# mbzuai-metaverse/XMem2

Hardware: AMD Instinct MI355X
Metric: frames/sec at 480p, 1 obj, 32 memory frames; mask IoU vs reference (higher is better)
Workload: dtype f32

## Files before the change

### include/xmem_hip.h

```cpp
#ifndef XMEM_HIP_H
#define XMEM_HIP_H

#include <stddef.h>
#include <stdint.h>

#ifdef __cplusplus
extern "C" {
#endif

typedef enum {
    XMEM_OK = 0,
    XMEM_ERR_BAD_ARG = -1,
    XMEM_ERR_UNSUPPORTED = -2,
    XMEM_ERR_WORKSPACE = -3,
    XMEM_ERR_LAUNCH = -4,
    XMEM_ERR_TOPK = -5
} xmem_status;

#define XMEM_ABI_VERSION 4
int xmem_version(void);
const char* xmem_last_error_string(int code);

int xmem_trace_marker(int tag, void* stream);

// ... 29 lines not shown
    int stream, ring;
} xmem_conv_plan_info;
int xmem_conv2d_plan_info(const xmem_conv_desc* d, xmem_conv_plan_info* out);

int xmem_conv2d_nhwc(const xmem_conv_desc* d, void* workspace, size_t workspace_bytes, void* stream);

#define XMEM_DILATED_NO_TAP_SKIP 1
size_t xmem_conv2d_dilated_workspace_bytes(const xmem_conv_desc* d, int dilation);
int xmem_conv2d_nhwc_dilated(const xmem_conv_desc* d, int dilation, int flags, void* workspace, size_t workspace_bytes, void* stream);

enum { XMEM_AUG_BRIGHTNESS = 0, XMEM_AUG_POSTERIZE = 1, XMEM_AUG_GRAY = 2, XMEM_AUG_SHARPNESS = 3, XMEM_AUG_BLUR7 = 4, XMEM_AUG_AFFINE = 5 };
#define XMEM_AUG_MAX 32
typedef struct {
    int type;
    float factor;
    double image_matrix[6];
    float mask_grid[6];
} xmem_aug_desc;
size_t xmem_augment_workspace_bytes(int n_aug, int H, int W);
int xmem_augment_frames(const uint8_t* img, const float* mask, int H, int W, int K, const xmem_aug_desc* descs, int n_aug,
                        uint8_t* out_img, float* out_mask, void* workspace, size_t workspace_bytes, void* stream);

int xmem_maxpool3x3s2(const float* in, float* out, int B, int H, int W, int C, void* stream);

int xmem_upsample2x_add(const float* g, const float* skip, float* out, int B, int h, int w, int C, void* stream);

int xmem_area_downsample(const float* in, int ldin, float* out, int ldout, int B, int H, int W, int C, int r, void* stream);

int xmem_copy_channels(const float* src, int ldsrc, int srcB, float* dst, int lddst, int B, int P, int C, void* stream);

int xmem_hidden_update_gather(const float* g16, int c16, const float* g8, int c8, const float* g4, int c4, const float* logits,
                              float* out, int ldout, int K, int h, int w, void* stream);

size_t xmem_cbam_workspace_bytes(int B, int P, int C);
int xmem_cbam_residual(const float* g, float* out, int B, int H, int W, int C,
                       const float* w1, const float* b1, const float* w2, const float* b2,
                       const float* sw, const float* sb, void* workspace, size_t workspace_bytes, void* stream);

int xmem_gru_gate(const float* values, const float* h, float* new_h, int B, int P, int Ch, void* stream);

int xmem_add3(const float* a, const float* b, const float* c, float* y, size_t n, void* stream);

int xmem_maxpool3x3s2_t(const void* in, int in_half, void* out, int out_half, int B, int H, int W, int C, void* stream);
int xmem_upsample2x_add_t(const void* g, const void* skip, void* out, int half, int B, int h, int w, int C, void* stream);
int xmem_area_downsample_t(const void* in, int in_half, int ldin, void* out, int out_half, int ldout, int B, int H, int W, int C, int r, void* stream);
int xmem_copy_channels_t(const void* src, int src_half, int ldsrc, int srcB, void* dst, int dst_half, int lddst, int B, int P, int C, void* stream);
int xmem_cbam_residual_t(const void* g, void* out, int half, int B, int H, int W, int C,
                         const float* w1, const float* b1, const float* w2, const float* b2,
                         const float* sw, const float* sb, void* workspace, size_t workspace_bytes, void* stream);
int xmem_gru_gate_t(const void* values, int values_half, const float* h, float* new_h, int B, int P, int Ch, void* stream);

int xmem_pack_image(const float* img, float* out, int H, int W, int Hp, int Wp, int lh, int lw, void* stream);

int xmem_pack_image_u8(const uint8_t* img, float* out, int H, int W, int Hp, int Wp, int lh, int lw,
                       const float* mean3_host, const float* std3_host, void* stream);

int xmem_pack_value_input(const float* image4, const float* masks, float* out, int K, int Hp, int Wp, void* stream);

int xmem_key_post(const float* proj, int ldp, float* key, float* shrinkage, float* selection, int P, int Ck, void* stream);

int xmem_logits_to_prob(const float* logits, float* prob, float* prob_padded, int K, int h4, int w4,
                        int H, int W, int lh, int lw, void* stream);

int xmem_aggregate_masks(const float* masks, float* prob, int K, int H, int W, void* stream);

int xmem_merge_masks(const float* pred_no_bg, const float* mask, uint64_t valid_bits, float* out, int K, int H, int W, void* stream);
// ... 106 lines not shown
```

### xmem2_amd/_lib.py

```python
import ctypes as C
import os

import torch

_HERE = os.path.dirname(os.path.abspath(__file__))
LIB_PATH = os.path.join(_HERE, 'csrc', 'libxmem_hip.so')
_lib = None

c_float_p = C.c_void_p
c_void_p = C.c_void_p


ABI_VERSION = 4


class ConvDesc(C.Structure):
    _fields_ = [('inp', C.c_void_p), ('B', C.c_int), ('H', C.c_int), ('W', C.c_int), ('Cin', C.c_int), ('ldin', C.c_int),
                ('w', C.c_void_p), ('Cout', C.c_int), ('KH', C.c_int), ('KW', C.c_int), ('stride', C.c_int), ('pad', C.c_int),
                ('scale', C.c_void_p), ('shift', C.c_void_p),
                ('res', C.c_void_p), ('ldres', C.c_int),
                ('out', C.c_void_p), ('ldout', C.c_int),
                ('relu_in', C.c_int), ('relu_out', C.c_int), ('plan_tile', C.c_int), ('plan_splitk', C.c_int), ('w_winograd', C.c_void_p),
                ('res_broadcast', C.c_int), ('w_winograd_f16', C.c_void_p), ('w_winograd4', C.c_void_p),
                ('arith', C.c_int), ('w_split', C.c_void_p), ('w_winograd_split', C.c_void_p), ('w_winograd4_split', C.c_void_p),
# ... 18 lines not shown


class AffinityHint(C.Structure):
    _fields_ = [('idx', C.c_void_p), ('top_k', C.c_int), ('n_seg', C.c_int), ('seg_n', C.c_int * 4), ('grid_w', C.c_int)]


class ValueSegment(C.Structure):
    _fields_ = [('value', C.c_void_p), ('n', C.c_int)]


_SIGS = {
    'xmem_version': (C.c_int, []),
    'xmem_last_error_string': (C.c_char_p, [C.c_int]),
    'xmem_trace_marker': (C.c_int, [C.c_int, C.c_void_p]),
    'xmem_conv2d_workspace_bytes': (C.c_size_t, [C.POINTER(ConvDesc)]),
    'xmem_conv2d_plan_info': (C.c_int, [C.POINTER(ConvDesc), C.POINTER(ConvPlanInfo)]),
    'xmem_conv2d_nhwc': (C.c_int, [C.POINTER(ConvDesc), C.c_void_p, C.c_size_t, C.c_void_p]),
    'xmem_conv2d_dilated_workspace_bytes': (C.c_size_t, [C.POINTER(ConvDesc), C.c_int]),
    'xmem_conv2d_nhwc_dilated': (C.c_int, [C.POINTER(ConvDesc), C.c_int, C.c_int, C.c_void_p, C.c_size_t, C.c_void_p]),
    'xmem_maxpool3x3s2': (C.c_int, [C.c_void_p, C.c_void_p, C.c_int, C.c_int, C.c_int, C.c_int, C.c_void_p]),
    'xmem_maxpool3x3s2_t': (C.c_int, [C.c_void_p, C.c_int, C.c_void_p, C.c_int, C.c_int, C.c_int, C.c_int, C.c_int, C.c_void_p]),
    'xmem_upsample2x_add_t': (C.c_int, [C.c_void_p, C.c_void_p, C.c_void_p, C.c_int, C.c_int, C.c_int, C.c_int, C.c_int, C.c_void_p]),
    'xmem_area_downsample_t': (C.c_int, [C.c_void_p, C.c_int, C.c_int, C.c_void_p, C.c_int, C.c_int, C.c_int, C.c_int, C.c_int, C.c_int, C.c_int, C.c_void_p]),
    'xmem_copy_channels_t': (C.c_int, [C.c_void_p, C.c_int, C.c_int, C.c_int, C.c_void_p, C.c_int, C.c_int, C.c_int, C.c_int, C.c_int, C.c_void_p]),
    'xmem_cbam_residual_t': (C.c_int, [C.c_void_p, C.c_void_p, C.c_int, C.c_int, C.c_int, C.c_int, C.c_int,
                                       C.c_void_p, C.c_void_p, C.c_void_p, C.c_void_p, C.c_void_p, C.c_void_p,
                                       C.c_void_p, C.c_size_t, C.c_void_p]),
    'xmem_gru_gate_t': (C.c_int, [C.c_void_p, C.c_int, C.c_void_p, C.c_void_p, C.c_int, C.c_int, C.c_int, C.c_void_p]),
    'xmem_upsample2x_add': (C.c_int, [C.c_void_p, C.c_void_p, C.c_void_p, C.c_int, C.c_int, C.c_int, C.c_int, C.c_void_p]),
    'xmem_area_downsample': (C.c_int, [C.c_void_p, C.c_int, C.c_void_p, C.c_int, C.c_int, C.c_int, C.c_int, C.c_int, C.c_int, C.c_void_p]),
    'xmem_copy_channels': (C.c_int, [C.c_void_p, C.c_int, C.c_int, C.c_void_p, C.c_int, C.c_int, C.c_int, C.c_int, C.c_void_p]),
    'xmem_hidden_update_gather': (C.c_int, [C.c_void_p, C.c_int, C.c_void_p, C.c_int, C.c_void_p, C.c_int, C.c_void_p, C.c_void_p, C.c_int, C.c_int, C.c_int,
                                            C.c_int, C.c_void_p]),
    'xmem_cbam_workspace_bytes': (C.c_size_t, [C.c_int, C.c_int, C.c_int]),
    'xmem_cbam_residual': (C.c_int, [C.c_void_p, C.c_void_p, C.c_int, C.c_int, C.c_int, C.c_int,
                                     C.c_void_p, C.c_void_p, C.c_void_p, C.c_void_p, C.c_void_p, C.c_void_p,
                                     C.c_void_p, C.c_size_t, C.c_void_p]),
    'xmem_gru_gate': (C.c_int, [C.c_void_p, C.c_void_p, C.c_void_p, C.c_int, C.c_int, C.c_int, C.c_void_p]),
    'xmem_add3': (C.c_int, [C.c_void_p, C.c_void_p, C.c_void_p, C.c_void_p, C.c_size_t, C.c_void_p]),
    'xmem_pack_image': (C.c_int, [C.c_void_p, C.c_void_p, C.c_int, C.c_int, C.c_int, C.c_int, C.c_int, C.c_int, C.c_void_p]),
    'xmem_pack_image_u8': (C.c_int, [C.c_void_p, C.c_void_p, C.c_int, C.c_int, C.c_int, C.c_int, C.c_int, C.c_int,
                                     C.POINTER(C.c_float), C.POINTER(C.c_float), C.c_void_p]),
    'xmem_pack_value_input': (C.c_int, [C.c_void_p, C.c_void_p, C.c_void_p, C.c_int, C.c_int, C.c_int, C.c_void_p]),
    'xmem_key_post': (C.c_int, [C.c_void_p, C.c_int, C.c_void_p, C.c_void_p, C.c_void_p, C.c_int, C.c_int, C.c_void_p]),
    'xmem_logits_to_prob': (C.c_int, [C.c_void_p, C.c_void_p, C.c_void_p, C.c_int, C.c_int, C.c_int, C.c_int, C.c_int, C.c_int, C.c_int, C.c_void_p]),
    'xmem_aggregate_masks': (C.c_int, [C.c_void_p, C.c_void_p, C.c_int, C.c_int, C.c_int, C.c_void_p]),
    'xmem_merge_masks': (C.c_int, [C.c_void_p, C.c_void_p, C.c_uint64, C.c_void_p, C.c_int, C.c_int, C.c_int, C.c_void_p]),
    'xmem_resize_bilinear': (C.c_int, [C.c_void_p, C.c_void_p, C.c_int, C.c_int, C.c_int, C.c_int, C.c_int, C.c_void_p]),
    'xmem_argmax_u8': (C.c_int, [C.c_void_p, C.c_void_p, C.c_int, C.c_int, C.c_int, C.c_void_p]),
    'xmem_ensemble_accumulate': (C.c_int, [C.c_void_p, C.c_int, C.c_int, C.c_int, C.c_int, C.c_void_p, C.c_int, C.c_int, C.c_int,
                                           C.c_void_p, C.c_void_p]),
    'xmem_jf_counts': (C.c_int, [C.c_void_p, C.c_void_p, C.c_void_p, C.c_int, C.c_int, C.c_int, C.c_int, C.c_void_p, C.c_void_p]),
    'xmem_s2m_pack': (C.c_int, [C.c_void_p, C.c_void_p, C.c_void_p, C.c_int, C.c_int, C.c_int, C.c_int, C.c_int, C.c_int, C.c_int,
                                C.c_int, C.c_void_p, C.c_void_p]),
    'xmem_channel_mean': (C.c_int, [C.c_void_p, C.c_int, C.c_int, C.c_int, C.c_int, C.c_void_p, C.c_void_p]),
    'xmem_broadcast_channels': (C.c_int, [C.c_void_p, C.c_void_p, C.c_int, C.c_int, C.c_int, C.c_int, C.c_void_p]),
    'xmem_resize_bilinear_nhwc': (C.c_int, [C.c_void_p, C.c_int, C.c_int, C.c_int, C.c_int, C.c_int, C.c_void_p, C.c_int, C.c_int,
                                            C.c_int, C.c_void_p]),
    'xmem_s2m_output': (C.c_int, [C.c_void_p, C.c_int, C.c_int, C.c_int, C.c_int, C.c_int, C.c_int, C.c_int, C.c_void_p, C.c_void_p,
                                  C.c_void_p, C.c_float, C.c_void_p]),
    'xmem_aggregate_wbg': (C.c_int, [C.c_void_p, C.c_int, C.c_int, C.c_int, C.c_int, C.c_float, C.c_void_p, C.c_void_p, C.c_void_p]),
    'xmem_nhwc_to_nchw': (C.c_int, [C.c_void_p, C.c_int, C.c_void_p, C.c_int, C.c_int, C.c_int, C.c_void_p]),
    'xmem_nchw_to_nhwc': (C.c_int, [C.c_void_p, C.c_void_p, C.c_int, C.c_int, C.c_int, C.c_int, C.c_void_p]),
    'xmem_affinity_topk_workspace_bytes': (C.c_size_t, [C.c_int, C.c_int, C.c_int]),
    'xmem_affinity_debug_offsets': (C.c_int, [C.c_int, C.c_int, C.POINTER(C.c_size_t), C.POINTER(C.c_size_t), C.POINTER(C.c_size_t)]),
    'xmem_augment_workspace_bytes': (C.c_size_t, [C.c_int, C.c_int, C.c_int]),
# ... 70 lines not shown
```

### xmem2_amd/csrc/conv_mfma.hip

```cpp
#include "common.hpp"
#include "gemm_stream.hpp"
#include <stdlib.h>


struct ConvArgs {
    const float* in; const float* w; const float* scale; const float* shift; const float* res;
    float* out; float* partial;
    int B, H, W, Cin, ldin;
    int Ho, Wo, Cout, ldout, ldres;
    int KH, KW, stride, pad;
    int K, M, HoWo;
    int relu_in, relu_out;
    int nk, splitk, kt_per_split;
    int tiles_m, tiles_n;
    int raw;
    int res_mod;
    long in_gstride, w_gstride, out_gstride;
    int a_presplit;
    int dbg;
    int dil, skip_taps;
};
#ifdef XMEM_TOOLS
#define CDBG(bit) (p.dbg & (bit))
#define CTRACE_MAX 16384
// ... 510 lines not shown
        }
#pragma unroll
        for (int t = 0; t < 9; ++t) wv[t] = *reinterpret_cast<const f32x4*>(p.w + (size_t)t * p.Cin + c);
        if (p.relu_in) {
#pragma unroll
            for (int r = 0; r < 3; ++r)
#pragma unroll
                for (int cc = 0; cc < 6; ++cc) {
                    f32x4& x = xv[r][cc];
                    x.x = fmaxf(x.x, 0.f); x.y = fmaxf(x.y, 0.f); x.z = fmaxf(x.z, 0.f); x.w = fmaxf(x.w, 0.f);
                }
        }
#pragma unroll
        for (int j = 0; j < 4; ++j)
#pragma unroll
            for (int t = 0; t < 9; ++t) {
                const int r = t / 3, cc = j + t % 3;
                if (!(okr[r] && okc[cc])) continue;
                const f32x4 x = xv[r][cc];
                acc[j] = fmaf(x.x, wv[t].x, acc[j]); acc[j] = fmaf(x.y, wv[t].y, acc[j]);
                acc[j] = fmaf(x.z, wv[t].z, acc[j]); acc[j] = fmaf(x.w, wv[t].w, acc[j]);
            }
    }
#pragma unroll
    for (int j = 0; j < 4; ++j) acc[j] = wave_sum(acc[j]);
    if (lane < 4 && ow0 + lane < p.Wo) {
        const float a = lane == 0 ? acc[0] : lane == 1 ? acc[1] : lane == 2 ? acc[2] : acc[3];
        const int m = row * p.Wo + ow0 + lane;
        float v = a * p.scale[0] + p.shift[0];
        if (p.res) v += p.res[(size_t)(p.res_mod ? m % p.res_mod : m) * p.ldres];
        if (p.relu_out) v = fmaxf(v, 0.f);
        p.out[(size_t)m * p.ldout] = v;
    }
}

__global__ void wino_input_kernel(const float* __restrict__ in, int ldin, int B, int H, int W, int C, int th, int tw,
                                  int relu_in, float* __restrict__ V, int split) {
    const int C4 = C >> 2;
    const size_t P = (size_t)B * th * tw;
    const size_t total = P * C4;
    for (size_t e = (size_t)blockIdx.x * blockDim.x + threadIdx.x; e < total; e += (size_t)gridDim.x * blockDim.x) {
        const int c4 = (int)(e % C4);
        size_t t = e / C4;
        const int tx = (int)(t % tw); size_t r = t / tw;
        const int ty = (int)(r % th);
        const int b = (int)(r / th);
        f32x4 d[4][4];
#pragma unroll
        for (int i = 0; i < 4; ++i) {
            const int ih = 2 * ty - 1 + i;
#pragma unroll
            for (int j = 0; j < 4; ++j) {
                const int iw = 2 * tx - 1 + j;
                f32x4 v = {0.f, 0.f, 0.f, 0.f};
                if ((unsigned)ih < (unsigned)H && (unsigned)iw < (unsigned)W)
                    v = *reinterpret_cast<const f32x4*>(in + (((size_t)b * H + ih) * W + iw) * ldin + c4 * 4);
                d[i][j] = v;
            }
        }
        if (relu_in) {
#pragma unroll
            for (int i = 0; i < 4; ++i)
#pragma unroll
                for (int j = 0; j < 4; ++j) {
                    f32x4 v = d[i][j];
                    v.x = fmaxf(v.x, 0.f); v.y = fmaxf(v.y, 0.f); v.z = fmaxf(v.z, 0.f); v.w = fmaxf(v.w, 0.f);
// ... 902 lines not shown
        g.M = a.M; g.N = d->Cout; g.K = d->Cin; g.G = 1;
        g.lda = d->ldin; g.ldb = d->Cin; g.ldc = d->ldout; g.ldres = d->ldres;
        g.mode = 1; g.relu_in = d->relu_in; g.relu_out = d->relu_out; g.res_mod = a.res_mod;
        g.stride = d->stride; g.H = d->H; g.W = d->W; g.Wo = Wo; g.HoWo = Ho * Wo;
        return gemm_stream_launch(g, stream_variant(pl), pl.ring, s);
    }
    if (pl.form == GEMV) {
        if (half) hipLaunchKernelGGL(conv_cout1_kernel<true>, dim3(cdiv(a.M, 4)), dim3(256), 0, s, a);
        else if (a.M >= 8192 && a.KH == 3 && a.KW == 3 && a.stride == 1 && a.Cin <= 256 && a.Ho == a.H + 2 * a.pad - 2 && a.Wo == a.W + 2 * a.pad - 2)
            hipLaunchKernelGGL(conv_cout1_row4_kernel, dim3(cdiv(a.B * a.Ho * ((a.Wo + 3) / 4), 4)), dim3(256), 0, s, a);
        else hipLaunchKernelGGL(conv_cout1_kernel<false>, dim3(cdiv(a.M, 4)), dim3(256), 0, s, a);
        return xmem_check_launch();
    }
    if ((rc = launch_tile(pl, a, s)) != XMEM_OK) return rc;
#ifdef XMEM_TOOLS
    if (a.dbg & 8) {
        static int printed = 0;
        (void)hipStreamSynchronize(s);
        const int n = a.tiles_m * a.tiles_n < CTRACE_MAX ? a.tiles_m * a.tiles_n : CTRACE_MAX;
        static unsigned long long h[CTRACE_MAX][6];
        (void)hipMemcpyFromSymbol(h, HIP_SYMBOL(g_conv_trace), sizeof(unsigned long long) * 6 * n);
        if (printed++ % 16 == 4) {
            double d[6] = {0, 0, 0, 0, 0, 0}; unsigned long long tmin = ~0ull, tmax = 0;
            for (int i = 0; i < n; ++i) { for (int k = 1; k < 6; ++k) d[k] += (double)(h[i][k] - h[i][0]); if (h[i][0] < tmin) tmin = h[i][0]; if (h[i][5] > tmax) tmax = h[i][5]; }
            fprintf(stderr, "[conv trace] %d workgroups: entry -> first tiles requested %.0f, in LDS %.0f, k-loop done %.0f, stores issued %.0f, stores landed %.0f ticks (mean); "
                            "first entry -> last store landed %.0f ticks; ticks are s_memtime units (100 MHz = 10 ns on gfx950)\n", n, d[1] / n, d[2] / n, d[3] / n, d[4] / n, d[5] / n,
                    (double)(tmax - tmin));
        }
    }
#endif
    return pl.splitk > 1 ? launch_splitk_reduce(a, half == 2, s) : rc;
}

namespace {

int validate_dilated(const xmem_conv_desc* d, int dilation) {
    const int rc = validate(d, dilation, 6);
    if (rc != XMEM_OK) return rc;
    if (d->Cout == 1 || d->in_half || d->out_half || d->arith != 0 || d->res_broadcast) return XMEM_ERR_UNSUPPORTED;
    if ((long)dilation * (d->KH - 1) > (1 << 20) || (long)dilation * (d->KW - 1) > (1 << 20)) return XMEM_ERR_UNSUPPORTED;
    return XMEM_OK;
}

Plan make_plan_dilated(const xmem_conv_desc* d, int dilation) {
    xmem_conv_desc v = *d;
    v.H = d->H - (dilation - 1) * (d->KH - 1);
    v.W = d->W - (dilation - 1) * (d->KW - 1);
    v.w_winograd = nullptr; v.w_winograd4 = nullptr; v.w_winograd_f16 = nullptr; v.w_split = nullptr; v.arith = 0;
    return make_plan(&v, v.plan_tile);
}

}

extern "C" size_t xmem_conv2d_dilated_workspace_bytes(const xmem_conv_desc* d, int dilation) {
    if (validate_dilated(d, dilation) != XMEM_OK) return 0;
    int Ho, Wo; out_dims(d, dilation, Ho, Wo);
    return splitk_workspace(make_plan_dilated(d, dilation), d, Ho, Wo);
}

extern "C" int xmem_conv2d_nhwc_dilated(const xmem_conv_desc* d, int dilation, int flags, void* workspace, size_t workspace_bytes,
                                        void* stream) {
    int rc = validate_dilated(d, dilation);
    if (rc != XMEM_OK) return rc;
    if (flags & ~XMEM_DILATED_NO_TAP_SKIP) return XMEM_ERR_BAD_ARG;
    const Plan pl = make_plan_dilated(d, dilation);
    int Ho, Wo; out_dims(d, dilation, Ho, Wo);
// ... 12 lines not shown
```

### xmem2_amd/network.py

```python
import collections
import os
import warnings
import weakref

import torch

from . import ops
from .arch import BN_EPS, infer_dims, state_dict_spec
from .ops import ConvWeights


def _pad4(n):
    return (n + 3) // 4 * 4


MAX_STAGES = 160


def _padc(n):
    return (n + 7) // 8 * 8 if ops.act_dtype() == torch.float16 else _pad4(n)


class XMem:
    def __init__(self, config, model_path=None, map_location=None, pretrained_key_encoder=True, pretrained_value_encoder=True):
        self.single_object = config.get('single_object', False)
        self.device = torch.device('cuda', torch.cuda.current_device()) if torch.cuda.is_available() else torch.device('cpu')
        self._sd = None
        self._w = {}
        self._cbam = {}
        self.use_graphs = os.environ.get('XMEM_HIP_GRAPHS', '1') != '0'
        self.precision = config.get('precision', os.environ.get('XMEM_PRECISION', 'fp32'))
        if self.precision not in ops.PRECISIONS:
            raise ValueError(f"config['precision'] must be one of {ops.PRECISIONS}, got {self.precision!r}")
        self._stages = collections.OrderedDict()
        self._zeros = {}
        self._owner_free, self._owner_next = [], 0
        self._call_precision = None
        self._scope = ops.new_scope()
        weakref.finalize(self, ops.release_scope, self._scope)
        weights = self.init_hyperparameters(config, model_path, map_location)
        if weights is not None:
            self.load_weights(weights, init_as_zero_if_needed=True)

    def init_hyperparameters(self, config, model_path=None, map_location=None):
        if model_path is not None:
            weights = torch.load(model_path, map_location=map_location or 'cpu', weights_only=True)
            self.key_dim, self.value_dim, self.hidden_dim = infer_dims(weights)
            self.disable_hidden = self.hidden_dim == 0
        else:
            weights = None
            self.key_dim = config.get('key_dim', 64)
            self.value_dim = config.get('value_dim', 512)
            self.hidden_dim = config.get('hidden_dim', 64)
            self.disable_hidden = self.hidden_dim <= 0
        config['key_dim'], config['value_dim'], config['hidden_dim'] = self.key_dim, self.value_dim, self.hidden_dim
        return weights

    def load_weights(self, src_dict, init_as_zero_if_needed=False):
        src_dict = dict(src_dict)
        k = 'value_encoder.conv1.weight'
        if k in src_dict and src_dict[k].shape[1] == 4 and not self.single_object:
            pads = torch.zeros((64, 1, 7, 7), device=src_dict[k].device)
            if not init_as_zero_if_needed:
# ... 98 lines not shown
            group_res(p + '.block1')
            group_res(p + '.block2')
            a = p + '.attention'
            dev = self.device
            self._cbam[a] = dict(
                w1=sd[a + '.ChannelGate.mlp.1.weight'].float().contiguous().to(dev),
                b1=sd[a + '.ChannelGate.mlp.1.bias'].float().contiguous().to(dev),
                w2=sd[a + '.ChannelGate.mlp.3.weight'].float().contiguous().to(dev),
                b2=sd[a + '.ChannelGate.mlp.3.bias'].float().contiguous().to(dev),
                sw=sd[a + '.SpatialGate.spatial.conv.weight'].float().reshape(2, 7, 7).contiguous().to(dev),
                sb=sd[a + '.SpatialGate.spatial.conv.bias'].float().contiguous().to(dev))

        fusion('value_encoder.fuser')
        fusion('decoder.fuser')

        def split_shared(name, x_dim=1024):
            cw = W[name]
            ones, zeros = torch.ones_like(cw.scale), torch.zeros_like(cw.shift)
            W[name + '@x'] = ConvWeights(cw.w[..., :x_dim].contiguous(), ones, zeros, cw.stride, cw.pad)
            W[name + '@g'] = ConvWeights(cw.w[..., x_dim:].contiguous(), cw.scale, cw.shift, cw.stride, cw.pad)

        for blk in ('value_encoder.fuser.block1', 'decoder.fuser.block1'):
            for c in ('.conv1', '.downsample'):
                if (blk + c) in W and W[blk + c].cin > 1024 and (W[blk + c].cin - 1024) % 32 == 0:
                    split_shared(blk + c)
        if self.hidden_dim > 0:
            W['value_encoder.hidden_reinforce.transform'] = self._conv_w('value_encoder.hidden_reinforce.transform', None, 1, 1)
            W['decoder.hidden_update.g16_conv'] = self._conv_w('decoder.hidden_update.g16_conv', None, 1, 0)
            W['decoder.hidden_update.g8_conv'] = self._conv_w('decoder.hidden_update.g8_conv', None, 1, 0)
            W['decoder.hidden_update.g4_conv'] = self._conv_w('decoder.hidden_update.g4_conv', None, 1, 0)
            W['decoder.hidden_update.transform'] = self._conv_w('decoder.hidden_update.transform', None, 1, 1)
            parts = [W['decoder.hidden_update.' + n] for n in ('g16_conv', 'g8_conv', 'g4_conv')]
            if all(float((p.scale - 1).abs().max()) == 0.0 for p in parts):
                wk = torch.cat([p.w for p in parts], 3).contiguous()
                W['decoder.hidden_update.g_fused'] = ConvWeights(wk, parts[0].scale, (parts[0].shift + parts[1].shift + parts[2].shift).contiguous(),
                                                                 1, 0, cin_true=sum(p.cin_true for p in parts))
        W['decoder.up_16_8.skip_conv'] = self._conv_w('decoder.up_16_8.skip_conv', None, 1, 1)
        group_res('decoder.up_16_8.out_conv')
        W['decoder.up_8_4.skip_conv'] = self._conv_w('decoder.up_8_4.skip_conv', None, 1, 1)
        group_res('decoder.up_8_4.out_conv')
        W['decoder.pred'] = self._conv_w('decoder.pred', None, 1, 1)
        parts = [self._conv_w('key_proj.' + n, None, 1, 1) for n in ('key_proj', 'd_proj', 'e_proj')]
        wk = torch.cat([p.w for p in parts], 0)
        sc, sh = torch.cat([p.scale for p in parts], 0), torch.cat([p.shift for p in parts], 0)
        extra = _pad4(wk.shape[0]) - wk.shape[0]
        if extra:
            wk = torch.cat([wk, wk.new_zeros((extra,) + tuple(wk.shape[1:]))], 0)
            sc, sh = torch.cat([sc, sc.new_ones(extra)], 0), torch.cat([sh, sh.new_zeros(extra)], 0)
        W['key_proj'] = ConvWeights(wk.contiguous(), sc.contiguous(), sh.contiguous(), 1, 1, cin_true=parts[0].cin_true)
        self._w = W

    def _need_weights(self):
        if not self._w:
            if self._sd is None:
                warnings.warn('XMem: no checkpoint loaded - using the deterministic synthetic weights (xmem2_amd.synth)')
                from .synth import synthetic_state_dict
                self._sd = synthetic_state_dict(0, self.key_dim, self.value_dim, self.hidden_dim)
            if self.device.type != 'cuda':
                raise RuntimeError('xmem2_amd.XMem runs on an MI355X (HIP) device only; call .to("cuda") - there is no CPU path')
            self._upload()

    def _run_stage(self, name, key, inputs, fn, alias=(), mutates=()):
        prec = self._call_precision or self.precision
        if not self.use_graphs or ops.eager_only() or name in os.environ.get('XMEM_EAGER_STAGES', '').split(','):
            with ops.precision(prec):
                return fn(*inputs)
        full_key = (name, key, prec) + tuple(tuple(t.shape) if t is not None else None for t in inputs)
# ... 229 lines not shown
            out = self._run_stage('segment', (tuple(out_hw), tuple(pad_tl), bool(h_out), True, slot, owner),
                                  [f16, f8, f4, cat16, hidden, skips[0], skips[1], skips[2], skips[3]],
                                  lambda a, b, c, d, e, s8, s4, sx, dx: self._segment_eager(a, b, c, d, e, h_out, (s8, s4, sx, dx), g4d),
                                  alias=(0, 1, 2, 4, 5, 6, 7, 8) if self._is_stage_output(f16) else (4,), mutates=(4,))
        elif skips is not None:
            out = self._run_stage('segment', (tuple(out_hw), tuple(pad_tl), bool(h_out), True, slot, owner),
                                  [f16, f8, f4, cat16, hidden, skips[0], skips[1]],
                                  lambda a, b, c, d, e, s8, s4: self._segment_eager(a, b, c, d, e, h_out, (s8, s4), g4d),
                                  alias=(0, 1, 2, 4, 5, 6) if self._is_stage_output(f16) else (4,), mutates=(4,))
        else:
            out = self._run_stage('segment', (tuple(out_hw), tuple(pad_tl), bool(h_out), False, slot, owner),
                                  [f16, f8, f4, cat16, hidden],
                                  lambda a, b, c, d, e: self._segment_eager(a, b, c, d, e, h_out, None, g4d),
                                  alias=(0, 1, 2, 4) if self._is_stage_output(f16) else (4,), mutates=(4,))
        new_hidden, logits = out
        H, Wd = out_hw
        prob, prob_padded = ops.logits_to_prob(logits.view(K, 4 * h, 4 * w), H, Wd, pad_tl[0], pad_tl[1])
        return new_hidden, prob, prob_padded

    def _segment_eager(self, f16, f8, f4, cat16, hidden, h_out, skips=None, g4d=None):
        W = self._w
        K, h, w, _ = cat16.shape
        hd = self.hidden_dim
        pre = (skips[2], skips[3]) if (skips is not None and len(skips) >= 4) else None
        if pre is None and not self._shares_x('decoder.fuser', K):
            ops.copy_channels(f16, cat16, 0)
        if hd > 0:
            ops.copy_channels(hidden, cat16, 1024 + self.value_dim)
        g16 = self._fusion(cat16, 'decoder.fuser', x=f16, pre=pre)
        skip8 = skips[0] if skips is not None else ops.conv2d(f8, W['decoder.up_16_8.skip_conv'])
        g8 = self._group_res(ops.upsample2x_add(g16, skip8), 'decoder.up_16_8.out_conv')
        skip4 = skips[1] if skips is not None else ops.conv2d(f4, W['decoder.up_8_4.skip_conv'])
        g4 = self._group_res(ops.upsample2x_add(g8, skip4), 'decoder.up_8_4.out_conv')
        logits = ops.conv2d(g4, W['decoder.pred'], relu_in=True, out_dtype=torch.float32)
        new_hidden = None
        if h_out and hd > 0:
            c4 = g4.shape[3]
            gf = W.get('decoder.hidden_update.g_fused')
            if g4d is None:
                g4d = self._zero_scratch((K, h, w, _padc(c4 + 1)), g4.device, ops.act_dtype())
            if gf is not None and g4d.shape[3] == gf.cin and g4d.dtype == torch.float32:
                c16, c8, ld = g16.shape[3], g8.shape[3], g4d.shape[3]
                if all(t.is_contiguous() for t in (g16, g8, g4, logits)):
                    ops.hidden_update_gather(g16, g8, g4, logits, g4d)
                else:
                    ops.copy_channels(g16, g4d, 0)
                    ops.area_downsample(g8, 2, out=g4d, out_ld=ld, out_off=c16)
                    ops.area_downsample(g4, 4, out=g4d, out_ld=ld, out_off=c16 + c8)
                    ops.area_downsample(logits, 4, out=g4d, out_ld=ld, out_off=c16 + c8 + c4)
                mid = gf.cout
                cat = torch.empty((K, h, w, mid + hd), dtype=ops.act_dtype(), device=g4.device)
                ops.conv2d(g4d, gf, out=cat, out_ld=cat.shape[3])
            else:
                ops.area_downsample(g4, 4, out=g4d, out_ld=g4d.shape[3])
                ops.area_downsample(logits, 4, out=g4d, out_ld=g4d.shape[3], out_off=c4)
                g8d = ops.area_downsample(g8, 2)
                t = ops.conv2d(g16, W['decoder.hidden_update.g16_conv'])
                t = ops.conv2d(g8d, W['decoder.hidden_update.g8_conv'], res=t)
                mid = t.shape[3]
                cat = torch.empty((K, h, w, mid + hd), dtype=ops.act_dtype(), device=g4.device)
                ops.conv2d(g4d, W['decoder.hidden_update.g4_conv'], res=t, out=cat, out_ld=cat.shape[3])
            ops.copy_channels(hidden, cat, mid)
            values = ops.conv2d(cat, W['decoder.hidden_update.transform'])
            new_hidden = ops.gru_gate(values, hidden, out=hidden)
        return new_hidden, logits

    @staticmethod
    def _as_nhwc(t):
        p = t.permute(0, 2, 3, 1)
        return p if p.is_contiguous() else ops.nchw_to_nhwc(t)

    def encode_key(self, frame, need_sk=True, need_ek=True):
        if frame.dim() != 4:
            raise NotImplementedError
        B, _, H, Wd = frame.shape
        image4 = torch.cat([ops.pack_image(frame[b], H, Wd, 0, 0) for b in range(B)], 0) if B > 1 \
            else ops.pack_image(frame[0], H, Wd, 0, 0)
        key, shr, sel, f16, f8, f4 = self.encode_key_nhwc(image4, need_sk, need_ek)
        h, w = f16.shape[1], f16.shape[2]
        nchw = lambda t: t.permute(0, 3, 1, 2)
        key = nchw(key.view(B, h, w, self.key_dim))
        shr = shr.view(B, 1, h, w) if shr is not None else None
        sel = nchw(sel.view(B, h, w, self.key_dim)) if sel is not None else None
        self._last_image4 = (frame.data_ptr(), image4)
        return key, shr, sel, nchw(f16), nchw(f8), nchw(f4)

    def encode_value(self, frame, image_feat_f16, h16, masks, is_deep_update=True):
        cached = getattr(self, '_last_image4', None)
        if cached is not None and cached[0] == frame.data_ptr():
            image4 = cached[1]
        else:
            image4 = ops.pack_image(frame[0], frame.shape[2], frame.shape[3], 0, 0)
        f16 = self._as_nhwc(image_feat_f16)
        hidden = self._as_nhwc(h16[0]) if h16 is not None else None
        m = masks[0] if masks[0].is_contiguous() else masks[0].contiguous()
        value, hidden = self.encode_value_nhwc(image4, f16, hidden, m, is_deep_update)
        value = value.permute(0, 3, 1, 2).unsqueeze(0)
        hidden = hidden.permute(0, 3, 1, 2).unsqueeze(0) if hidden is not None else None
# ... 33 lines not shown
```

### xmem2_amd/ops.py

```python
import contextlib
import ctypes as C
import math
import os
import threading

import torch

from . import _lib, conv_plan
from ._lib import AffinityHint, ConvDesc, KeySegment, ValueSegment, check, load, ptr, stream_ptr

_workspaces = {}
_retired = {}
_tls = threading.local()
_scope_free, _scope_next = [], [0]


def new_scope():
    if _scope_free:
        return _scope_free.pop()
    _scope_next[0] += 1
    return _scope_next[0]


@contextlib.contextmanager
# ... 396 lines not shown
def area_downsample(x, r, out=None, out_ld=None, out_off=0, c=None, in_ld=None):
    B, H, W = x.shape[:3]
    c = c if c is not None else x.shape[3]
    in_ld = in_ld if in_ld is not None else x.shape[3]
    if out is None:
        out = torch.empty((B, H // r, W // r, c), dtype=x.dtype, device=x.device)
        out_ld = c
    check(load().xmem_area_downsample_t(ptr(x), _h(x), in_ld, C.c_void_p(out.data_ptr() + out.element_size() * out_off), _h(out), out_ld,
                                        B, H, W, c, r, stream_ptr()))
    return out


def copy_channels(src, dst, dst_off, c=None, src_off=0):
    B = dst.shape[0]
    P = dst.shape[1] * dst.shape[2]
    c = c if c is not None else src.shape[3]
    check(load().xmem_copy_channels_t(C.c_void_p(src.data_ptr() + src.element_size() * src_off), _h(src), src.shape[3], src.shape[0],
                                      C.c_void_p(dst.data_ptr() + dst.element_size() * dst_off), _h(dst), dst.shape[3], B, P, c, stream_ptr()))
    return dst


def hidden_update_gather(g16, g8, g4, logits, out):
    K, h, w, c16 = g16.shape
    if any(t.dtype != torch.float32 or not t.is_contiguous() for t in (g16, g8, g4, logits, out)):
        raise RuntimeError('hidden_update_gather: contiguous float32 tensors only')
    if tuple(g8.shape[:3]) != (K, 2 * h, 2 * w) or tuple(g4.shape[:3]) != (K, 4 * h, 4 * w) or tuple(logits.shape) != (K, 4 * h, 4 * w, 1) \
            or tuple(out.shape[:3]) != (K, h, w):
        raise RuntimeError('hidden_update_gather: shapes do not belong to one decoder pass')
    check(load().xmem_hidden_update_gather(ptr(g16), c16, ptr(g8), g8.shape[3], ptr(g4), g4.shape[3], ptr(logits), ptr(out), out.shape[3],
                                           K, h, w, stream_ptr()))
    return out


def cbam_residual(g, p):
    lib = load()
    B, H, W, Cc = g.shape
    out = torch.empty_like(g)
    need = lib.xmem_cbam_workspace_bytes(B, H * W, Cc)
    ws = workspace(need, g.device, 'cbam')
    check(lib.xmem_cbam_residual_t(ptr(g), ptr(out), _h(g), B, H, W, Cc, ptr(p['w1']), ptr(p['b1']), ptr(p['w2']), ptr(p['b2']),
                                   ptr(p['sw']), ptr(p['sb']), ptr(ws), need, stream_ptr()))
    return out


def gru_gate(values, h, out=None):
    B, H, W, Ch = h.shape
    if out is None:
        out = torch.empty_like(h)
    check(load().xmem_gru_gate_t(ptr(values), _h(values), ptr(h), ptr(out), B, H * W, Ch, stream_ptr()))
    return out


def pack_image(img, Hp, Wp, lh, lw, out=None):
    _req(img, 'image')
    if not img.is_contiguous():
        img = img.contiguous()
    if out is None:
        out = torch.empty((1, Hp, Wp, 4), dtype=torch.float32, device=img.device)
    check(load().xmem_pack_image(ptr(img), ptr(out), img.shape[1], img.shape[2], Hp, Wp, lh, lw, stream_ptr()))
    return out


IM_MEAN = (0.485, 0.456, 0.406)
IM_STD = (0.229, 0.224, 0.225)


# ... 352 lines not shown
```

Before: 658.2.

## Fuse mask-head 3x3 conv with hidden-update gather and downsampling into one kernel

Adds a fused HIP kernel that, per 1/16-resolution pixel, computes the Cout=1 3x3 mask-prediction conv over a 4x4 patch of g4. In the same pass it writes the area-downsampled g4/g8/logit features and copies g16 and hidden into the hidden-update input buffers. This replaces the separate pred conv, the gather/downsample launches and repeated reads of g4. It also pads the fused g-conv weights to a multiple of 32 input channels and pins a plan for the unpadded path. In exchange it adds a specialised fp32-only path gated by shape checks and a minimum pixel count, and changes the summation order of the logits.

```diff
diff --git a/include/xmem_hip.h b/include/xmem_hip.h
--- a/include/xmem_hip.h
+++ b/include/xmem_hip.h
@@ -85,6 +85,10 @@
 int xmem_hidden_update_gather(const float* g16, int c16, const float* g8, int c8, const float* g4, int c4, const float* logits,
                               float* out, int ldout, int K, int h, int w, void* stream);
 
+int xmem_mask_head_gather(const float* g16, int c16, const float* g8, int c8, const float* g4, int c4, const float* w,
+                          const float* scale, const float* shift, const float* hidden, int hd, float* logits, float* g4d,
+                          int ldg4d, float* cat, int ldcat, int K, int h, int wd, void* stream);
+
 size_t xmem_cbam_workspace_bytes(int B, int P, int C);
 int xmem_cbam_residual(const float* g, float* out, int B, int H, int W, int C,
                        const float* w1, const float* b1, const float* w2, const float* b2,
diff --git a/xmem2_amd/_lib.py b/xmem2_amd/_lib.py
--- a/xmem2_amd/_lib.py
+++ b/xmem2_amd/_lib.py
@@ -74,6 +74,9 @@
     'xmem_copy_channels': (C.c_int, [C.c_void_p, C.c_int, C.c_int, C.c_void_p, C.c_int, C.c_int, C.c_int, C.c_int, C.c_void_p]),
     'xmem_hidden_update_gather': (C.c_int, [C.c_void_p, C.c_int, C.c_void_p, C.c_int, C.c_void_p, C.c_int, C.c_void_p, C.c_void_p, C.c_int, C.c_int, C.c_int,
                                             C.c_int, C.c_void_p]),
+    'xmem_mask_head_gather': (C.c_int, [C.c_void_p, C.c_int, C.c_void_p, C.c_int, C.c_void_p, C.c_int, C.c_void_p, C.c_void_p, C.c_void_p,
+                                        C.c_void_p, C.c_int, C.c_void_p, C.c_void_p, C.c_int, C.c_void_p, C.c_int, C.c_int, C.c_int, C.c_int,
+                                        C.c_void_p]),
     'xmem_cbam_workspace_bytes': (C.c_size_t, [C.c_int, C.c_int, C.c_int]),
     'xmem_cbam_residual': (C.c_int, [C.c_void_p, C.c_void_p, C.c_int, C.c_int, C.c_int, C.c_int,
                                      C.c_void_p, C.c_void_p, C.c_void_p, C.c_void_p, C.c_void_p, C.c_void_p,
diff --git a/xmem2_amd/csrc/conv_mfma.hip b/xmem2_amd/csrc/conv_mfma.hip
--- a/xmem2_amd/csrc/conv_mfma.hip
+++ b/xmem2_amd/csrc/conv_mfma.hip
@@ -566,6 +566,119 @@
         if (p.relu_out) v = fmaxf(v, 0.f);
         p.out[(size_t)m * p.ldout] = v;
     }
+}
+
+struct MaskTailArgs {
+    const float *g16, *g8, *g4, *w, *scale, *shift, *hidden;
+    float *logits, *g4d, *cat;
+    int c16, c8, c4, hd, ldg, ldcat, K, h, wd;
+};
+
+__global__ __launch_bounds__(64, 2) void conv_cout1_tail_kernel(MaskTailArgs p) {
+    const int lane = threadIdx.x;
+    const size_t pix = blockIdx.x;
+    const int x = (int)(pix % p.wd); const size_t ky = pix / p.wd;
+    const int y = (int)(ky % p.h);
+    const int W4 = 4 * p.wd;
+    const int c = lane * 4;
+    const bool act = c < p.c4;
+    const bool okr0 = y > 0, okr5 = y < p.h - 1, okc0 = x > 0, okc5 = x < p.wd - 1;
+    f32x4 xv[6][6], wv[9];
+    const float sc = p.scale[0], sf = p.shift[0];
+    if (act) {
+        const float* base = p.g4 + ((4 * ky) * (size_t)W4 + 4 * x) * p.c4 + c;
+        const long rowl = (long)W4 * p.c4;
+#pragma unroll
+        for (int r = 0; r < 6; ++r) {
+            const long ro = (r == 0 ? (okr0 ? -1 : 0) : r == 5 ? (okr5 ? 4 : 3) : r - 1) * rowl;
+#pragma unroll
+            for (int cc = 0; cc < 6; ++cc) {
+                const long co = (long)(cc == 0 ? (okc0 ? -1 : 0) : cc == 5 ? (okc5 ? 4 : 3) : cc - 1) * p.c4;
+                xv[r][cc] = *reinterpret_cast<const f32x4*>(base + ro + co);
+            }
+        }
+#pragma unroll
+        for (int t = 0; t < 9; ++t) wv[t] = *reinterpret_cast<const f32x4*>(p.w + (size_t)t * p.c4 + c);
+    }
+    const int n16 = p.c16 >> 2, n8 = p.c8 >> 2, nh = p.hd >> 2;
+    float* const o = p.g4d + pix * p.ldg;
+    float* const oh = p.cat + pix * p.ldcat;
+    const float* const s16 = p.g16 + pix * p.c16;
+    const float* const s8 = p.g8 + ((2 * ky) * (size_t)(2 * p.wd) + 2 * x) * p.c8;
+    const float* const sh = p.hidden + pix * p.hd;
+    const size_t row8 = (size_t)(2 * p.wd) * p.c8;
+    const bool a0 = lane < n16, a1 = lane + 64 < n16, b0 = lane < n8, h0 = lane < nh;
+    f32x4 va0, va1, vb[4], vh;
+    if (a0) va0 = *reinterpret_cast<const f32x4*>(s16 + 4 * lane);
+    if (a1) va1 = *reinterpret_cast<const f32x4*>(s16 + 4 * (lane + 64));
+    if (h0) vh = *reinterpret_cast<const f32x4*>(sh + 4 * lane);
+    if (b0) {
+        const float* src = s8 + 4 * lane;
+        vb[0] = *reinterpret_cast<const f32x4*>(src); vb[1] = *reinterpret_cast<const f32x4*>(src + p.c8);
+        vb[2] = *reinterpret_cast<const f32x4*>(src + row8); vb[3] = *reinterpret_cast<const f32x4*>(src + row8 + p.c8);
+    }
+    float acc[16];
+#pragma unroll
+    for (int j = 0; j < 16; ++j) acc[j] = 0.f;
+    if (act) {
+        f32x4 s = {0.f, 0.f, 0.f, 0.f};
+#pragma unroll
+        for (int dy = 0; dy < 4; ++dy)
+#pragma unroll
+            for (int dx = 0; dx < 4; ++dx) s += xv[1 + dy][1 + dx];
+        *reinterpret_cast<f32x4*>(p.g4d + pix * p.ldg + p.c16 + p.c8 + c) = s * 0.0625f;
+#pragma unroll
+        for (int r = 0; r < 6; ++r)
+#pragma unroll
+            for (int cc = 0; cc < 6; ++cc) {
+                f32x4& v = xv[r][cc];
+                v.x = fmaxf(v.x, 0.f); v.y = fmaxf(v.y, 0.f); v.z = fmaxf(v.z, 0.f); v.w = fmaxf(v.w, 0.f);
+            }
+#pragma unroll
+        for (int j = 0; j < 16; ++j)
+#pragma unroll
+            for (int t = 0; t < 9; ++t) {
+                const int r = (j >> 2) + t / 3, cc = (j & 3) + t % 3;
+                if ((r == 0 && !okr0) || (r == 5 && !okr5) || (cc == 0 && !okc0) || (cc == 5 && !okc5)) continue;
+                const f32x4 v = xv[r][cc];
+                acc[j] = fmaf(v.x, wv[t].x, acc[j]); acc[j] = fmaf(v.y, wv[t].y, acc[j]);
+                acc[j] = fmaf(v.z, wv[t].z, acc[j]); acc[j] = fmaf(v.w, wv[t].w, acc[j]);
+            }
+    }
+    if (a0) *reinterpret_cast<f32x4*>(o + 4 * lane) = va0;
+    if (a1) *reinterpret_cast<f32x4*>(o + 4 * (lane + 64)) = va1;
+    if (b0) {
+        f32x4 s = {0.f, 0.f, 0.f, 0.f};
+        s += vb[0]; s += vb[1]; s += vb[2]; s += vb[3];
+        *reinterpret_cast<f32x4*>(o + p.c16 + 4 * lane) = s * 0.25f;
+    }
+    if (h0) *reinterpret_cast<f32x4*>(oh + 4 * lane) = vh;
+    float lsum = 0.f;
+#pragma unroll
+    for (int j = 0; j < 16; ++j) {
+        const float a = wave_sum(acc[j]);
+        acc[j] = a * sc + sf;
+        lsum += acc[j];
+    }
+    if (lane < 4) {
+        f32x4 v;
+        v.x = lane == 0 ? acc[0] : lane == 1 ? acc[4] : lane == 2 ? acc[8] : acc[12];
+        v.y = lane == 0 ? acc[1] : lane == 1 ? acc[5] : lane == 2 ? acc[9] : acc[13];
+        v.z = lane == 0 ? acc[2] : lane == 1 ? acc[6] : lane == 2 ? acc[10] : acc[14];
+        v.w = lane == 0 ? acc[3] : lane == 1 ? acc[7] : lane == 2 ? acc[11] : acc[15];
+        *reinterpret_cast<f32x4*>(p.logits + (4 * ky + lane) * (size_t)W4 + 4 * x) = v;
+    }
+    if (lane == 4) p.g4d[pix * p.ldg + p.c16 + p.c8 + p.c4] = lsum * 0.0625f;
+    for (int g = lane + 128; g < n16; g += 64) *reinterpret_cast<f32x4*>(o + 4 * g) = *reinterpret_cast<const f32x4*>(s16 + 4 * g);
+    for (int g = lane + 64; g < n8; g += 64) {
+        const float* src = s8 + 4 * g;
+        const f32x4 q0 = *reinterpret_cast<const f32x4*>(src), q1 = *reinterpret_cast<const f32x4*>(src + p.c8);
+        const f32x4 q2 = *reinterpret_cast<const f32x4*>(src + row8), q3 = *reinterpret_cast<const f32x4*>(src + row8 + p.c8);
+        f32x4 s = {0.f, 0.f, 0.f, 0.f};
+        s += q0; s += q1; s += q2; s += q3;
+        *reinterpret_cast<f32x4*>(o + p.c16 + 4 * g) = s * 0.25f;
+    }
+    for (int g = lane + 64; g < nh; g += 64) *reinterpret_cast<f32x4*>(oh + 4 * g) = *reinterpret_cast<const f32x4*>(sh + 4 * g);
 }
 
 __global__ void wino_input_kernel(const float* __restrict__ in, int ldin, int B, int H, int W, int C, int th, int tw,
@@ -1534,6 +1647,24 @@
     return pl.splitk > 1 ? launch_splitk_reduce(a, half == 2, s) : rc;
 }
 
+extern "C" int xmem_mask_head_gather(const float* g16, int c16, const float* g8, int c8, const float* g4, int c4, const float* w,
+                                     const float* scale, const float* shift, const float* hidden, int hd, float* logits, float* g4d,
+                                     int ldg4d, float* cat, int ldcat, int K, int h, int wd, void* stream) {
+    if (!g16 || !g8 || !g4 || !w || !scale || !shift || !hidden || !logits || !g4d || !cat) return XMEM_ERR_BAD_ARG;
+    if (K <= 0 || h <= 0 || wd <= 0 || c16 <= 0 || c8 <= 0 || c4 <= 0 || hd <= 0) return XMEM_ERR_BAD_ARG;
+    if (c16 % 4 || c8 % 4 || c4 % 4 || hd % 4 || ldg4d % 4 || ldcat % 4 || c4 > 256) return XMEM_ERR_UNSUPPORTED;
+    if (ldg4d < c16 + c8 + c4 + 1 || ldcat < hd) return XMEM_ERR_UNSUPPORTED;
+    if (((uintptr_t)g16 | (uintptr_t)g8 | (uintptr_t)g4 | (uintptr_t)w | (uintptr_t)hidden | (uintptr_t)logits | (uintptr_t)g4d | (uintptr_t)cat) & 15)
+        return XMEM_ERR_UNSUPPORTED;
+    if ((double)K * h * wd >= 2.0e9 / 16) return XMEM_ERR_UNSUPPORTED;
+    MaskTailArgs a;
+    a.g16 = g16; a.g8 = g8; a.g4 = g4; a.w = w; a.scale = scale; a.shift = shift; a.hidden = hidden;
+    a.logits = logits; a.g4d = g4d; a.cat = cat;
+    a.c16 = c16; a.c8 = c8; a.c4 = c4; a.hd = hd; a.ldg = ldg4d; a.ldcat = ldcat; a.K = K; a.h = h; a.wd = wd;
+    hipLaunchKernelGGL(conv_cout1_tail_kernel, dim3(K * h * wd), dim3(64), 0, reinterpret_cast<hipStream_t>(stream), a);
+    return xmem_check_launch();
+}
+
 namespace {
 
 int validate_dilated(const xmem_conv_desc* d, int dilation) {
diff --git a/xmem2_amd/network.py b/xmem2_amd/network.py
--- a/xmem2_amd/network.py
+++ b/xmem2_amd/network.py
@@ -15,6 +15,7 @@
 
 
 MAX_STAGES = 160
+FUSED_TAIL_MIN_PIXELS = 512
 
 
 def _padc(n):
@@ -29,6 +30,8 @@
         self._w = {}
         self._cbam = {}
         self.use_graphs = os.environ.get('XMEM_HIP_GRAPHS', '1') != '0'
+        self.fused_tail = os.environ.get('XMEM_FUSED_TAIL', '1') != '0'
+        self.fused_tail_min_pixels = FUSED_TAIL_MIN_PIXELS
         self.precision = config.get('precision', os.environ.get('XMEM_PRECISION', 'fp32'))
         if self.precision not in ops.PRECISIONS:
             raise ValueError(f"config['precision'] must be one of {ops.PRECISIONS}, got {self.precision!r}")
@@ -193,7 +196,10 @@
             W['decoder.hidden_update.transform'] = self._conv_w('decoder.hidden_update.transform', None, 1, 1)
             parts = [W['decoder.hidden_update.' + n] for n in ('g16_conv', 'g8_conv', 'g4_conv')]
             if all(float((p.scale - 1).abs().max()) == 0.0 for p in parts):
-                wk = torch.cat([p.w for p in parts], 3).contiguous()
+                wk = torch.cat([p.w for p in parts], 3)
+                if self.fused_tail and wk.shape[3] % 32:
+                    wk = torch.nn.functional.pad(wk, (0, 32 - wk.shape[3] % 32))
+                wk = wk.contiguous()
                 W['decoder.hidden_update.g_fused'] = ConvWeights(wk, parts[0].scale, (parts[0].shift + parts[1].shift + parts[2].shift).contiguous(),
                                                                  1, 0, cin_true=sum(p.cin_true for p in parts))
         W['decoder.up_16_8.skip_conv'] = self._conv_w('decoder.up_16_8.skip_conv', None, 1, 1)
@@ -489,11 +495,20 @@
         g8 = self._group_res(ops.upsample2x_add(g16, skip8), 'decoder.up_16_8.out_conv')
         skip4 = skips[1] if skips is not None else ops.conv2d(f4, W['decoder.up_8_4.skip_conv'])
         g4 = self._group_res(ops.upsample2x_add(g8, skip4), 'decoder.up_8_4.out_conv')
+        gf = W.get('decoder.hidden_update.g_fused') if h_out and hd > 0 else None
+        if self.fused_tail and gf is not None and g4d is not None and g4d.shape[3] == gf.cin and K * h * w >= self.fused_tail_min_pixels \
+                and hidden.shape[3] == hd:
+            mid = gf.cout
+            cat = torch.empty((K, h, w, mid + hd), dtype=torch.float32, device=g4.device)
+            if ops.mask_head_gather_ok(g16, g8, g4, W['decoder.pred'], hidden, g4d, cat, mid):
+                logits = ops.mask_head_gather(g16, g8, g4, W['decoder.pred'], hidden, g4d, cat, mid)
+                ops.conv2d(g4d, gf, out=cat, out_ld=cat.shape[3])
+                values = ops.conv2d(cat, W['decoder.hidden_update.transform'])
+                return ops.gru_gate(values, hidden, out=hidden), logits
         logits = ops.conv2d(g4, W['decoder.pred'], relu_in=True, out_dtype=torch.float32)
         new_hidden = None
         if h_out and hd > 0:
             c4 = g4.shape[3]
-            gf = W.get('decoder.hidden_update.g_fused')
             if g4d is None:
                 g4d = self._zero_scratch((K, h, w, _padc(c4 + 1)), g4.device, ops.act_dtype())
             if gf is not None and g4d.shape[3] == gf.cin and g4d.dtype == torch.float32:
@@ -507,7 +522,7 @@
                     ops.area_downsample(logits, 4, out=g4d, out_ld=ld, out_off=c16 + c8 + c4)
                 mid = gf.cout
                 cat = torch.empty((K, h, w, mid + hd), dtype=ops.act_dtype(), device=g4.device)
-                ops.conv2d(g4d, gf, out=cat, out_ld=cat.shape[3])
+                ops.conv2d(g4d, gf, out=cat, out_ld=cat.shape[3], plan=self._unpadded_g_fused_plan(gf, K, h, w, cat.shape[3]))
             else:
                 ops.area_downsample(g4, 4, out=g4d, out_ld=g4d.shape[3])
                 ops.area_downsample(logits, 4, out=g4d, out_ld=g4d.shape[3], out_off=c4)
@@ -521,6 +536,14 @@
             values = ops.conv2d(cat, W['decoder.hidden_update.transform'])
             new_hidden = ops.gru_gate(values, hidden, out=hidden)
         return new_hidden, logits
+
+    @staticmethod
+    def _unpadded_g_fused_plan(gf, K, h, w, out_ld):
+        from . import conv_plan
+        if gf.cin % 32 == 0 or ops._PRECISION != 'fp32' or conv_plan.CONV_FORM or conv_plan.AUTOTUNE:
+            return None
+        cp = (gf.cin + 31) // 32 * 32
+        return conv_plan.FP32.get(f'{K}x{h}x{w}x{cp}/{cp}->{gf.cout}/{out_ld} k1s1p0 r000')
 
     @staticmethod
     def _as_nhwc(t):
diff --git a/xmem2_amd/ops.py b/xmem2_amd/ops.py
--- a/xmem2_amd/ops.py
+++ b/xmem2_amd/ops.py
@@ -452,6 +452,39 @@
     return out
 
 
+def mask_head_gather_ok(g16, g8, g4, cw, hidden, g4d, cat, cat_off):
+    ts = (g16, g8, g4, hidden, g4d, cat)
+    if _PRECISION != 'fp32' or any(t is None or t.dtype != torch.float32 or not t.is_contiguous() for t in ts):
+        return False
+    K, h, w, c16 = g16.shape
+    c8, c4, hd = g8.shape[3], g4.shape[3], hidden.shape[3]
+    return (tuple(g8.shape[:3]) == (K, 2 * h, 2 * w) and tuple(g4.shape[:3]) == (K, 4 * h, 4 * w)
+            and tuple(hidden.shape[:3]) == (K, h, w) and tuple(g4d.shape[:3]) == (K, h, w) and tuple(cat.shape[:3]) == (K, h, w)
+            and (cw.cout, cw.kh, cw.kw, cw.stride, cw.pad, cw.dilation, cw.cin) == (1, 3, 3, 1, 1, 1, c4) and c4 <= 256
+            and not (c16 % 4 or c8 % 4 or c4 % 4 or hd % 4 or cat_off % 4 or cat.shape[3] % 4 or g4d.shape[3] % 4)
+            and g4d.shape[3] >= c16 + c8 + c4 + 1 and cat_off + hd <= cat.shape[3])
+
+
+def mask_head_gather(g16, g8, g4, cw, hidden, g4d, cat, cat_off):
+    if not mask_head_gather_ok(g16, g8, g4, cw, hidden, g4d, cat, cat_off):
+        raise RuntimeError('mask_head_gather: float32 mode, contiguous float32 tensors of one decoder pass and a 3x3 mask head over <= 256 channels only')
+    K, h, w, c16 = g16.shape
+    c8, c4, hd = g8.shape[3], g4.shape[3], hidden.shape[3]
+    logits = torch.empty((K, 4 * h, 4 * w, 1), dtype=torch.float32, device=g4.device)
+    dst = C.c_void_p(cat.data_ptr() + 4 * cat_off)
+    launch = lambda: load().xmem_mask_head_gather(ptr(g16), c16, ptr(g8), c8, ptr(g4), c4, ptr(cw.w), ptr(cw.scale), ptr(cw.shift),
+                                                  ptr(hidden), hd, ptr(logits), ptr(g4d), g4d.shape[3], dst, cat.shape[3], K, h, w,
+                                                  stream_ptr())
+    check(launch())
+    if RECORD is not None:
+        H, W = 4 * h, 4 * w
+        key = f'{K}x{H}x{W}x{c4}/{c4}->1/1 k3s1p1 r010'
+        RECORD.append(('conv', key, 2.0 * K * H * W * 9 * cw.cin_true, launch,
+                       (g4, logits, None, cw, None, dict(relu_in=True, relu_out=False, in_ld=c4, cin=c4, out_ld=1, res_broadcast=False,
+                                                         plan=(conv_plan.HEURISTIC, 0), executed_mfma_flops=0.0))))
+    return logits
+
+
 def cbam_residual(g, p):
     lib = load()
     B, H, W, Cc = g.shape
```

New measurement: 666.2, median of 6. 1.2% higher.
